# JGasp/alphazero-risk

Hardware: AMD Instinct MI355X
Metric: MCTS simulations/s (higher is better)
Workload: dtype bf16

## Files before the change

alphazero-risk_amd/csrc/azr_tower_sb.hip:

```cpp
#include <stdlib.h>
#include <string.h>

#include "azr_internal.hpp"
#include "azr_tower_common.hpp"

using namespace azr;

namespace {
constexpr int NT = 4;
constexpr int WAVES = 4, THREADS = 256;

template <int NB_>
struct SB {
    static constexpr int NB = NB_;
    static constexpr int ROWS = 42 * NB;
    static constexpr int MT = (ROWS + 15) / 16;
    static constexpr int ZR = MT * 16;
    static constexpr int RING = 4;
    static constexpr int BUF = (ZR + 1) * ROWB;
    static constexpr int FEAT_OFF = BUF;
    static constexpr int HEAD_OFF = FEAT_OFF + (ZR + 1) * FROWB;
    using TAB = TowerTables<NB, ZR, HEAD_OFF + NB * 448 * 4>;
    static constexpr int FOLD_OFF = TAB::END;
    static constexpr int LDS_BYTES = FOLD_OFF + 2 * NF * 4;
    static_assert(NB >= 2 && NB <= 4, "tile shapes");
    static_assert(72 % RING == 0 && RING <= MAX_RING, "ring depth");
    static_assert(LDS_BYTES <= 160 * 1024, "LDS budget");
    static_assert(BUF % 16 == 0 && FEAT_OFF % 16 == 0 && HEAD_OFF % 16 == 0 && FOLD_OFF % 16 == 0, "alignment");
    static_assert(3 * NF * 4 <= (ZR + 1) * FROWB, "the heads stage 3 x 256 floats in the stem feature image");
};

template <int N>
__device__ __forceinline__ void wait_lgkm()
{
    if constexpr (N >= 0 && N <= 14) __builtin_amdgcn_s_waitcnt(0xC07F | (N << 8));
}

template <int NB, int TAP, bool F16>
__device__ __forceinline__ void conv_tap(const uint8_t* bufX, const uint8_t* tr_c, uint32_t g16, const __amdgpu_buffer_rsrc_t wsrc,
                                         uint32_t loff, uint32_t& wk, u32x4 (&bq)[SB<NB>::RING][NT], f32x4 (&acc)[SB<NB>::MT][NT],
                                         s16x8 (&a)[SB<NB>::MT], uint32_t (&ap)[SB<NB>::MT])
{
    constexpr int MT = SB<NB>::MT, ZR = SB<NB>::ZR, RING = SB<NB>::RING;
    constexpr uint32_t sk = skip_mask<NB>(TAP), skn = skip_mask<NB>(TAP + 1);
    constexpr int active = MT - __builtin_popcount(sk & ((1u << MT) - 1u));
    uint32_t np[MT];
#pragma unroll
    for (int ks = 0; ks < KS_PER_TAP; ks++) {
        const int gk = TAP * KS_PER_TAP + ks;
        const int cur = gk % RING, ref = (gk + RING - 1) % RING;
        {
            constexpr int VM = (RING - 2) * NT;
            __builtin_amdgcn_s_waitcnt(0x0F70 | (VM & 15) | ((VM >> 4) << 14));
        }
#pragma unroll
        for (int mt = 0; mt < MT; mt++) {
            if (!((sk >> mt) & 1u)) {
                const int j = __builtin_popcount(~sk & ((1u << mt) - 1u));
                acc[mt][0] = El<F16>::mfma(bq[cur][0], a[mt], acc[mt][0]);
#pragma unroll
                for (int nt = 0; nt < NT; nt++)
                    if (j == ((nt + 1) * active) / NT - 1)
                        bq[ref][nt] = __builtin_amdgcn_raw_buffer_load_b128(wsrc, loff + nt * 1024, (int)(wk + (RING - 1) * KBYTES), 0);
                __builtin_amdgcn_sched_barrier(0);
                acc[mt][1] = El<F16>::mfma(bq[cur][1], a[mt], acc[mt][1]);
                wait_lgkm<active - 2>();
                __builtin_amdgcn_sched_barrier(0);
                acc[mt][2] = El<F16>::mfma(bq[cur][2], a[mt], acc[mt][2]);
                acc[mt][3] = El<F16>::mfma(bq[cur][3], a[mt], acc[mt][3]);
                if (ks < KS_PER_TAP - 1) a[mt] = lds16(bufX + ap[mt] + (ks + 1) * 64);
            }
            if (ks == KS_PER_TAP - 3) { if (!((skn >> mt) & 1u)) np[mt] = (uint32_t)tr_c[(TAP + 1) * ZR + mt * 16]; }
            if (ks == KS_PER_TAP - 2) { if (!((skn >> mt) & 1u)) np[mt] = np[mt] * ROWB + g16; }
            if (ks == KS_PER_TAP - 1) { if (!((skn >> mt) & 1u)) a[mt] = lds16(bufX + np[mt]); }
            __builtin_amdgcn_sched_barrier(0);
        }
        wk += (uint32_t)KBYTES;
    }
#pragma unroll
    for (int mt = 0; mt < MT; mt++) ap[mt] = np[mt];
}

template <int NB, bool F16>
__global__ __launch_bounds__(THREADS, 1) void k_tower_sb(const uint8_t* __restrict__ in88, int in_stride, int n,
                                                          const uint16_t* __restrict__ stem_wp, const uint16_t* __restrict__ tower_wp,
                                                          const float* __restrict__ fold, int blocks, const float* __restrict__ hp,
                                                          float* __restrict__ pi_out, float* __restrict__ v_out,
                                                          unsigned long long* __restrict__ diag, const int* __restrict__ slot_map)
{
    using G = SB<NB>;
    constexpr int ROWS = G::ROWS, MT = G::MT, ZR = G::ZR, RING = G::RING;
    extern __shared__ __attribute__((aligned(16))) uint8_t lds[];
    uint8_t* bufX = lds;
    uint8_t* bufF = lds + G::FEAT_OFF;
    uint8_t* in_l = lds + G::TAB::IN88_OFF;
    uint8_t* rowof = lds + G::TAB::ROWOF_OFF;
    uint8_t* taprow = lds + G::TAB::TAPROW_OFF;
    uint16_t* rowcell = reinterpret_cast<uint16_t*>(lds + G::TAB::ROWCELL_OFF);
    float* foldl = reinterpret_cast<float*>(lds + G::FOLD_OFF);
    const int tid = threadIdx.x, lane = tid & 63, wave = tid >> 6;
    const int c = lane & 15, g = lane >> 4;
    const int board0 = blockIdx.x * NB;
    if (diag && blockIdx.x == 0 && tid == 0) { diag[0] = __builtin_amdgcn_s_memtime(); diag[1] = __builtin_amdgcn_s_memrealtime(); }
    if (diag && tid == 0) {
        diag[8 + 8 * (size_t)blockIdx.x] = __builtin_amdgcn_s_memrealtime();
        diag[8 + 8 * (size_t)blockIdx.x + 4] = __builtin_amdgcn_s_getreg((20 ) | (0 << 6) | (3 << 11)) & 15u;
    }

    const __amdgpu_buffer_rsrc_t wsrc = __builtin_amdgcn_make_buffer_rsrc(const_cast<uint16_t*>(tower_wp), (short)0, 0x7fffffff, 0x00020000);
    const uint32_t loff = (uint32_t)((wave * NT) * 64 + lane) * 16u;
    uint32_t wk = 0;
    u32x4 bq[RING][NT];
#pragma unroll
    for (int ks = 0; ks < RING - 1; ks++)
#pragma unroll
        for (int nt = 0; nt < NT; nt++) bq[ks][nt] = __builtin_amdgcn_raw_buffer_load_b128(wsrc, loff + nt * 1024, ks * (int)KBYTES, 0);

    stage_inputs<NB, THREADS>(in_l, in88, in_stride, board0, n, slot_map);
    clear_zero_rows<THREADS>(bufX + ZR * ROWB);
    build_row_tables<NB, THREADS, 10>(rowof, taprow, rowcell);
    stem_features<ZR, THREADS>(in_l, rowcell, reinterpret_cast<uint16_t*>(bufF), [](float v) { return El<F16>::rne(v); });
    __syncthreads();

    f32x4 acc[MT][NT];
    uint2 res[MT][NT];
    const uint32_t eoff = (uint32_t)(c * ROWB + (wave * 64 + g * 4) * 2);

    {
#pragma unroll
        for (int mt = 0; mt < MT; mt++)
#pragma unroll
            for (int nt = 0; nt < NT; nt++) acc[mt][nt] = f32x4{0, 0, 0, 0};
        const s16x8* wp = reinterpret_cast<const s16x8*>(stem_wp) + (size_t)(wave * NT) * 64 + lane;
#pragma unroll
        for (int ks = 0; ks < STEM_KS; ks++) {
            const int tap = 2 * ks + (g >> 1);
            s16x8 b[NT];
#pragma unroll
            for (int nt = 0; nt < NT; nt++) b[nt] = wp[(size_t)ks * FRAGS_PER_KSTEP * 64 + nt * 64];
#pragma unroll
            for (int mt = 0; mt < MT; mt++) {
                const int row = taprow[tap * ZR + mt * 16 + c];
                const s16x8 av = lds16(bufF + row * FROWB + (g & 1) * 16);
#pragma unroll
                for (int nt = 0; nt < NT; nt++)
                    acc[mt][nt] = El<F16>::mfma(b[nt], av, acc[mt][nt]);
            }
        }
#pragma unroll
        for (int mt = 0; mt < MT; mt++) {
            const int ci = rowcell[mt * 16 + c];
            const int y = ci == 0xffff ? 0 : (ci & 15);
            const float sc = fold[y], sh = fold[7 + y];
#pragma unroll
            for (int nt = 0; nt < NT; nt++) {
                const uint2 o = bn_relu_pack<false, F16>(acc[mt][nt], float4{sc, sc, sc, sc}, float4{sh, sh, sh, sh}, uint2{0, 0});
                res[mt][nt] = o;
                if (c < pad_from<NB>(mt)) *reinterpret_cast<uint2*>(bufX + eoff + mt * 16 * ROWB + nt * 32) = o;
            }
        }
    }
    __syncthreads();

    if (diag && tid == 0) { diag[8 + 8 * (size_t)blockIdx.x + 1] = __builtin_amdgcn_s_memrealtime(); diag[8 + 8 * (size_t)blockIdx.x + 5] = __builtin_amdgcn_s_memtime(); }
    const uint8_t* tr_c = taprow + c;
    const uint32_t g16 = (uint32_t)g * 16u;
    const int layers = 2 * blocks;
    for (int L = 0; L < layers; L++) {
#pragma unroll
        for (int mt = 0; mt < MT; mt++)
#pragma unroll
            for (int nt = 0; nt < NT; nt++) acc[mt][nt] = f32x4{0, 0, 0, 0};
        const float2 fnext = *reinterpret_cast<const float2*>(fold + 14 + (size_t)L * 2 * NF + 2 * tid);
        uint32_t ap[MT];
        s16x8 a[MT];
        {
            const uint32_t sk0 = skip_mask<NB>(0);
#pragma unroll
            for (int mt = 0; mt < MT; mt++) {
                ap[mt] = (uint32_t)tr_c[mt * 16] * ROWB + g16;
                if (!((sk0 >> mt) & 1u)) a[mt] = lds16(bufX + ap[mt]);
            }
        }
        conv_tap<NB, 0, F16>(bufX, tr_c, g16, wsrc, loff, wk, bq, acc, a, ap);
        conv_tap<NB, 1, F16>(bufX, tr_c, g16, wsrc, loff, wk, bq, acc, a, ap);
        conv_tap<NB, 2, F16>(bufX, tr_c, g16, wsrc, loff, wk, bq, acc, a, ap);
        conv_tap<NB, 3, F16>(bufX, tr_c, g16, wsrc, loff, wk, bq, acc, a, ap);
        conv_tap<NB, 4, F16>(bufX, tr_c, g16, wsrc, loff, wk, bq, acc, a, ap);
        conv_tap<NB, 5, F16>(bufX, tr_c, g16, wsrc, loff, wk, bq, acc, a, ap);
        conv_tap<NB, 6, F16>(bufX, tr_c, g16, wsrc, loff, wk, bq, acc, a, ap);
        conv_tap<NB, 7, F16>(bufX, tr_c, g16, wsrc, loff, wk, bq, acc, a, ap);
        conv_tap<NB, 8, F16>(bufX, tr_c, g16, wsrc, loff, wk, bq, acc, a, ap);
        *reinterpret_cast<float2*>(foldl + 2 * tid) = fnext;
        __syncthreads();
        float4 sc[NT], sh[NT];
#pragma unroll
        for (int nt = 0; nt < NT; nt++) {
            sc[nt] = *reinterpret_cast<const float4*>(foldl + wave * 64 + g * 4 + nt * 16);
            sh[nt] = *reinterpret_cast<const float4*>(foldl + NF + wave * 64 + g * 4 + nt * 16);
        }
        int even = ~L & 1;
        asm volatile("" : "+s"(even));
        if (L & 1) {
#pragma unroll
            for (int mt = 0; mt < MT; mt++)
#pragma unroll
                for (int nt = 0; nt < NT; nt++) {
                    const uint2 o = bn_relu_pack<true, F16>(acc[mt][nt], sc[nt], sh[nt], res[mt][nt]);
                    res[mt][nt] = o;
                    if (c < pad_from<NB>(mt)) *reinterpret_cast<uint2*>(bufX + eoff + mt * 16 * ROWB + nt * 32) = o;
                }
        }
        if (even) {
#pragma unroll
            for (int mt = 0; mt < MT; mt++)
#pragma unroll
                for (int nt = 0; nt < NT; nt++) {
                    const uint2 o = bn_relu_pack<false, F16>(acc[mt][nt], sc[nt], sh[nt], uint2{0, 0});
                    if (c < pad_from<NB>(mt)) *reinterpret_cast<uint2*>(bufX + eoff + mt * 16 * ROWB + nt * 32) = o;
                }
        }
        __syncthreads();
    }

    if (diag && blockIdx.x == 0 && tid == 0) { diag[2] = __builtin_amdgcn_s_memtime(); diag[3] = __builtin_amdgcn_s_memrealtime(); }
    if (diag && tid == 0) { diag[8 + 8 * (size_t)blockIdx.x + 2] = __builtin_amdgcn_s_memrealtime(); diag[8 + 8 * (size_t)blockIdx.x + 6] = __builtin_amdgcn_s_memtime(); }
    fused_heads<NB, THREADS>(tid, hp, reinterpret_cast<float*>(bufF), reinterpret_cast<float*>(lds + G::HEAD_OFF), rowof, ImageAct<F16>{bufX},
                             board0, n, slot_map, pi_out, v_out);
    if (diag && tid == 0) diag[8 + 8 * (size_t)blockIdx.x + 3] = __builtin_amdgcn_s_memrealtime();
}
}

namespace azr {

template <int NB, bool F16> struct Shape { static constexpr int nb = NB; static constexpr bool f16 = F16; };
template <class Fn>
static int sb_dispatch(azr_engine* h, int nb, Fn f)
{
    if (bf16net(h)->f16) return nb == 4 ? f(Shape<4, true>{}) : nb == 3 ? f(Shape<3, true>{}) : f(Shape<2, true>{});
    return nb == 4 ? f(Shape<4, false>{}) : nb == 3 ? f(Shape<3, false>{}) : f(Shape<2, false>{});
}

int tower_sb_init(azr_engine* h)
{
    for (int nb = 4; nb >= 2; nb--) {
        const int rc = sb_dispatch(h, nb, [&](auto s) -> int {
            constexpr int NB = decltype(s)::nb;
            constexpr bool F16 = decltype(s)::f16;
            HIPCHK(h, hipFuncSetAttribute(reinterpret_cast<const void*>(k_tower_sb<NB, F16>), hipFuncAttributeMaxDynamicSharedMemorySize, SB<NB>::LDS_BYTES));
            return AZR_OK;
        });
        if (rc) return rc;
    }
    return AZR_OK;
}

int tower_sb_launch(azr_engine* h, int nb, int wgs, const uint8_t* d_in88, int in_stride, int n, float* d_pi, float* d_v, const int* d_map, hipStream_t st)
{
    if (nb < 2 || nb > 4 || wgs < 1 || (long long)wgs * nb < n) { h->err = "tower_sb_launch: bad tiling"; return AZR_E_INVALID_ARGUMENT; }
    Bf16Net* x = bf16net(h);
    sb_dispatch(h, nb, [&](auto s) {
        constexpr int NB = decltype(s)::nb;
        constexpr bool F16 = decltype(s)::f16;
        hipLaunchKernelGGL((k_tower_sb<NB, F16>), dim3(wgs), dim3(THREADS), SB<NB>::LDS_BYTES, st, d_in88, in_stride, n, x->stem_wp, x->tower_wp,
                           F16 ? (const float*)x->fold16 : net_fold(h), h->net.blocks, net_head_params(h), d_pi, d_v, x->diag, d_map);
        return 0;
    });
    HIPCHK(h, hipGetLastError());
    return AZR_OK;
}

}
```

Measured before the change: 962,000.

## Reorder conv tap MFMAs into nt-major groups with computed LDS waits

Restructures the inner convolution loop so MFMAs are issued in groups of GS row tiles sweeping across the N tiles, instead of all four N tiles per row tile. A constexpr Deal table decides where the weight prefetch buffer loads go and where LDS waitcnts are placed, so each A fragment's wait sits a fixed lead ahead of its first use. The goal is to spread the LDS and global loads more evenly between MFMAs and avoid back-to-back dependent MFMA chains on the same accumulator. The risk is wrong waitcnt counts or extra scheduling barriers that stall issue.

Result: no change. 966,800, median of 6 (+0.5%).

```diff
diff --git a/alphazero-risk_amd/csrc/azr_tower_sb.hip b/alphazero-risk_amd/csrc/azr_tower_sb.hip
--- a/alphazero-risk_amd/csrc/azr_tower_sb.hip
+++ b/alphazero-risk_amd/csrc/azr_tower_sb.hip
@@ -17,6 +17,7 @@
     static constexpr int MT = (ROWS + 15) / 16;
     static constexpr int ZR = MT * 16;
     static constexpr int RING = 4;
+    static constexpr int GS = NB == 3 ? 1 : 2;
     static constexpr int BUF = (ZR + 1) * ROWB;
     static constexpr int FEAT_OFF = BUF;
     static constexpr int HEAD_OFF = FEAT_OFF + (ZR + 1) * FROWB;
@@ -35,15 +36,54 @@
 {
     if constexpr (N >= 0 && N <= 14) __builtin_amdgcn_s_waitcnt(0xC07F | (N << 8));
 }
+__device__ __forceinline__ void wait_lgkm_n(int n)
+{
+#define AZR_W(N) case N: wait_lgkm<N>(); break;
+    switch (n) { AZR_W(0) AZR_W(1) AZR_W(2) AZR_W(3) AZR_W(4) AZR_W(5) AZR_W(6) AZR_W(7) AZR_W(8) AZR_W(9) AZR_W(10) AZR_W(11) AZR_W(12) AZR_W(13) AZR_W(14) default: break; }
+#undef AZR_W
+}
+
+constexpr int LEAD = 2;
+template <int MT, int GS>
+struct Deal {
+    int slot[NT] = {};
+    int wgap[MT] = {};
+    constexpr Deal(uint32_t on)
+    {
+        int sweep[MT * NT] = {}, total = 0;
+        for (int g0 = 0; g0 < MT; g0 += GS)
+            for (int nt = 0; nt < NT; nt++)
+                for (int mt = g0; mt < g0 + GS && mt < MT; mt++)
+                    if ((on >> mt) & 1u) {
+                        if (nt == 0) {
+                            int g = total - 1 - LEAD;
+                            while (g >= 0 && sweep[g] == 3) g--;
+                            wgap[mt] = g < 0 ? -1 : g;
+                        }
+                        sweep[total++] = nt;
+                    }
+        const int active = total / NT;
+        int last = -1;
+        for (int q = 0; q < NT; q++) {
+            int t = 4 * (((q + 1) * active) / NT - 1);
+            if (t <= last) t = last + 1;
+            int p = t;
+            while (p < total && sweep[p] == 3) p++;
+            if (p >= total) for (p = t; p > last + 1 && sweep[p] == 3;) p--;
+            slot[q] = last = p;
+        }
+    }
+};
 
 template <int NB, int TAP, bool F16>
 __device__ __forceinline__ void conv_tap(const uint8_t* bufX, const uint8_t* tr_c, uint32_t g16, const __amdgpu_buffer_rsrc_t wsrc,
                                          uint32_t loff, uint32_t& wk, u32x4 (&bq)[SB<NB>::RING][NT], f32x4 (&acc)[SB<NB>::MT][NT],
                                          s16x8 (&a)[SB<NB>::MT], uint32_t (&ap)[SB<NB>::MT])
 {
-    constexpr int MT = SB<NB>::MT, ZR = SB<NB>::ZR, RING = SB<NB>::RING;
-    constexpr uint32_t sk = skip_mask<NB>(TAP), skn = skip_mask<NB>(TAP + 1);
-    constexpr int active = MT - __builtin_popcount(sk & ((1u << MT) - 1u));
+    constexpr int MT = SB<NB>::MT, ZR = SB<NB>::ZR, RING = SB<NB>::RING, GS = SB<NB>::GS;
+    constexpr uint32_t full = (1u << MT) - 1u;
+    constexpr uint32_t on = ~skip_mask<NB>(TAP) & full, onn = ~skip_mask<NB>(TAP + 1) & full;
+    constexpr Deal<MT, GS> deal(on);
     uint32_t np[MT];
 #pragma unroll
     for (int ks = 0; ks < KS_PER_TAP; ks++) {
@@ -53,27 +93,51 @@
             constexpr int VM = (RING - 2) * NT;
             __builtin_amdgcn_s_waitcnt(0x0F70 | (VM & 15) | ((VM >> 4) << 14));
         }
-#pragma unroll
-        for (int mt = 0; mt < MT; mt++) {
-            if (!((sk >> mt) & 1u)) {
-                const int j = __builtin_popcount(~sk & ((1u << mt) - 1u));
-                acc[mt][0] = El<F16>::mfma(bq[cur][0], a[mt], acc[mt][0]);
-#pragma unroll
-                for (int nt = 0; nt < NT; nt++)
-                    if (j == ((nt + 1) * active) / NT - 1)
-                        bq[ref][nt] = __builtin_amdgcn_raw_buffer_load_b128(wsrc, loff + nt * 1024, (int)(wk + (RING - 1) * KBYTES), 0);
-                __builtin_amdgcn_sched_barrier(0);
-                acc[mt][1] = El<F16>::mfma(bq[cur][1], a[mt], acc[mt][1]);
-                wait_lgkm<active - 2>();
-                __builtin_amdgcn_sched_barrier(0);
-                acc[mt][2] = El<F16>::mfma(bq[cur][2], a[mt], acc[mt][2]);
-                acc[mt][3] = El<F16>::mfma(bq[cur][3], a[mt], acc[mt][3]);
-                if (ks < KS_PER_TAP - 1) a[mt] = lds16(bufX + ap[mt] + (ks + 1) * 64);
+        const uint32_t frd = ks < KS_PER_TAP - 1 ? on : onn;
+        const uint32_t tbl = ks == KS_PER_TAP - 3 ? onn : 0u, tblp = ks == KS_PER_TAP - 2 ? onn : 0u;
+        auto waits = [&](int g, uint32_t done) {
+#pragma unroll
+            for (int t = MT - 1; t >= 0; t--)
+                if (((on >> t) & 1u) && deal.wgap[t] == g) {
+                    const uint32_t above = full & ~((2u << t) - 1u);
+                    wait_lgkm_n(__builtin_popcount(on & above) + __builtin_popcount(tblp & (above | (1u << t))) +
+                                __builtin_popcount(frd & done) + __builtin_popcount(tbl & done));
+                    return true;
+                }
+            return false;
+        };
+        if (waits(-1, 0u)) __builtin_amdgcn_sched_barrier(0);
+        int m = 0;
+#pragma unroll
+        for (int g0 = 0; g0 < MT; g0 += GS) {
+#pragma unroll
+            for (int nt = 0; nt < NT; nt++) {
+#pragma unroll
+                for (int i = 0; i < GS; i++) {
+                    const int mt = g0 + i;
+                    if (mt >= MT) continue;
+                    bool piece = false;
+                    if ((on >> mt) & 1u) {
+                        acc[mt][nt] = El<F16>::mfma(bq[cur][nt], a[mt], acc[mt][nt]);
+#pragma unroll
+                        for (int q = 0; q < NT; q++)
+                            if (m == deal.slot[q]) {
+                                bq[ref][q] = __builtin_amdgcn_raw_buffer_load_b128(wsrc, loff + q * 1024, (int)(wk + (RING - 1) * KBYTES), 0);
+                                piece = true;
+                            }
+                        if (nt == NT - 1 && ks < KS_PER_TAP - 1) { a[mt] = lds16(bufX + ap[mt] + (ks + 1) * 64); piece = true; }
+                        if (waits(m, (1u << g0) - 1u)) piece = true;
+                        m++;
+                    }
+                    if (nt == NT - 1 && ((onn >> mt) & 1u)) {
+                        if (ks == KS_PER_TAP - 3) np[mt] = (uint32_t)tr_c[(TAP + 1) * ZR + mt * 16];
+                        if (ks == KS_PER_TAP - 2) np[mt] = np[mt] * ROWB + g16;
+                        if (ks == KS_PER_TAP - 1) a[mt] = lds16(bufX + np[mt]);
+                        piece = true;
+                    }
+                    if (piece) __builtin_amdgcn_sched_barrier(0);
+                }
             }
-            if (ks == KS_PER_TAP - 3) { if (!((skn >> mt) & 1u)) np[mt] = (uint32_t)tr_c[(TAP + 1) * ZR + mt * 16]; }
-            if (ks == KS_PER_TAP - 2) { if (!((skn >> mt) & 1u)) np[mt] = np[mt] * ROWB + g16; }
-            if (ks == KS_PER_TAP - 1) { if (!((skn >> mt) & 1u)) a[mt] = lds16(bufX + np[mt]); }
-            __builtin_amdgcn_sched_barrier(0);
         }
         wk += (uint32_t)KBYTES;
     }
```
